# pdeljanov/Symphonia

Hardware: AMD Instinct MI355X
Metric: decoded audio frames/sec (batch IMDCT+OLA) (higher is better)
Workload: dtype f32

## Files before the change

symphonia_amd/build.py:

```python
import hashlib
import json
import os
import shutil
import subprocess
import sys
from pathlib import Path

HERE = Path(__file__).resolve().parent
CSRC = HERE / "csrc"
OUT = HERE / "libsymaccel.so"
TUNED_OUT = HERE / "build" / "tuned" / "libsymaccel.so"
SOURCES = ["tables.cpp", "ctx.cpp", "host_tools.cpp", "stage.cpp", "batcher.cpp", "multi.cpp", "imdct_generic.hip", "imdct_big.hip", "aac.hip", "aac_tools.hip", "mp3.hip", "mpa_polyphase.hip", "mp3_requant.hip",
           "mp3_stereo.hip", "vorbis.hip", "vorbis_wave.hip", "vorbis_wave2.hip", "vorbis_wg.hip", "flac.hip", "alac.hip", "state_copy.hip", "batch_copy.hip", "probe.hip"]
ARCH = "gfx950"
FLAGS = ["-O3", "-std=c++17", "-fPIC", "-I", str(CSRC), "-ffp-contract=off", "-fno-fast-math", "-fno-slp-vectorize", "-Wall", "-Wno-unused-function",
         "-Wno-unused-variable", "-Wno-unused-but-set-variable", "-Wno-missing-braces"]
_ILP = ["-mllvm", "-amdgpu-sched-strategy=iterative-ilp"]
SOURCE_FLAGS = {"aac_tools.hip": _ILP, "mp3.hip": _ILP, "alac.hip": _ILP, "flac.hip": _ILP}
TUNING_KNOBS = ("AAC_MIN_WAVES", "AAC_PREFETCH", "AAC_VARIANT", "NT", "MP3_WAVES", "MP3_VARIANT", "MP3_WG_WAVES", "MP3_FUSED_WAVES", "MP3_FUSED_WG_WAVES", "VORBIS_WAVES", "ALAC_SMALL_WAVES", "FLAC_PARTS", "MP3_SLOT_GROUP", "MP3_PACKED", "MP3_PAIR_GROUP", "AAC_ABLATE", "AAC_SINK", "AAC_CLOCK", "AAC_QUAD", "MULTI_WAVE", "VORBIS_WAVE2", "VORBIS_WG", "VORBIS_WG_SHARED", "ST_POLICY", "PACKED_C32", "WG4096_ABLATE", "FLAC_STORE_SWITCH", "ALAC_ONE_LAUNCH", "MP3_FRONT", "LDS_ABLATE", "F1_ABLATE", "F1_WAVES", "TNS_AHEAD", "TNS_ABLATE", "ALAC_UPDATE", "FLAC_OLDEST_FIRST", "FLAC_GROUP", "ALAC_UNROLL", "F1_LANE16", "FLAC_WAVES")
TUNE_PREFIX = "SYMACCEL_TUNE_"


def hipcc():
    exe = shutil.which("hipcc") or "/opt/rocm/bin/hipcc"
    if not Path(exe).exists():
        raise RuntimeError("hipcc not found: libsymaccel has no CPU build")
    return exe


def tuned_source_flags(env=None):
    env = os.environ if env is None else env
    names = [n for n in env.get(TUNE_PREFIX + "ILP", "").split(",") if n]
    for n in names:
        if n not in SOURCES:
            raise ValueError("%sILP names %r, not one of the sources" % (TUNE_PREFIX, n))
    out = {k: list(v) for k, v in SOURCE_FLAGS.items()}
    for n in names:
        out[n] = ["-mllvm", "-amdgpu-sched-strategy=" + env.get(TUNE_PREFIX + "SCHED", "iterative-ilp")]
    return out


def tuning_defines(env=None):
# ... 115 lines not shown
```

symphonia_amd/csrc/aac.hip:

```cpp
#include <type_traits>

#include "imdct_wave.h"

namespace symaccel {

namespace {

#ifndef SYM_AAC_VARIANT
#define SYM_AAC_VARIANT 0
#endif
#if SYM_AAC_VARIANT == 1
constexpr int kWaves = 6;
#define SYM_AAC_WAVES_PER_SIMD 3
#else
constexpr int kWaves = 4;
#endif
constexpr int kTabTw = 0;
constexpr int kTabKbd = 1024;
constexpr int kTabSine = 2048;
constexpr int kTabKbdShort = 3072;
constexpr int kTabSineShort = 3200;
constexpr int kTabFloats = 3328;

enum : int { ONLY_LONG = 0, LONG_START = 1, EIGHT_SHORT = 2, LONG_STOP = 3 };
constexpr int kP0 = 512 - 64;
constexpr int kP1 = 512 + 64;

__device__ __forceinline__ void pcm_short4(const float *H, int q0, const float *short_win, const float *prev_short_win,
                                           float (&acc)[4]) {
    const int w = q0 >> 7, i0 = q0 & 127;
    bool have = false;
    if (w >= 1) {
        float a[4];
        ys4(H, w - 1, 128 + i0, a);
        const float4 wr = *reinterpret_cast<const float4 *>(short_win + 124 - i0);
        a[0] *= wr.w; a[1] *= wr.z; a[2] *= wr.y; a[3] *= wr.x;
#pragma unroll
        for (int q = 0; q < 4; ++q) acc[q] = (w - 1 == 0) ? a[q] : (0.0f + a[q]);
        have = true;
    }
    if (w <= 7) {
        float bq[4];
        ys4(H, w, i0, bq);
        const float4 wf = *reinterpret_cast<const float4 *>((w == 0 ? prev_short_win : short_win) + i0);
        bq[0] *= wf.x; bq[1] *= wf.y; bq[2] *= wf.z; bq[3] *= wf.w;
#pragma unroll
        for (int q = 0; q < 4; ++q) acc[q] = have ? (acc[q] + bq[q]) : bq[q];
    }
}

__device__ __forceinline__ void stop_window4(const float *psw, int j0, float *w) {
    float4 v = make_float4(1.0f, 1.0f, 1.0f, 1.0f);
    if (j0 >= kP0 && j0 < kP1) v = *reinterpret_cast<const float4 *>(psw + j0 - kP0);
    w[0] = v.x; w[1] = v.y; w[2] = v.z; w[3] = v.w;
}
__device__ __forceinline__ void start_window4(const float *sw, int j0, float *w) {
    float4 v = make_float4(1.0f, 1.0f, 1.0f, 1.0f);
    if (j0 >= kP0 && j0 < kP1) {
        const float4 r = *reinterpret_cast<const float4 *>(sw + 124 - (j0 - kP0));
        v = make_float4(r.w, r.z, r.y, r.x);
    }
    w[0] = v.x; w[1] = v.y; w[2] = v.z; w[3] = v.w;
}

#if defined(SYM_AAC_WAVES_PER_SIMD) && !defined(SYM_AAC_MIN_WAVES)
#define SYM_AAC_MIN_WAVES SYM_AAC_WAVES_PER_SIMD
#endif
#ifndef SYM_AAC_MIN_WAVES
#define SYM_AAC_MIN_WAVES 2
#endif
#ifndef SYM_AAC_PREFETCH
#define SYM_AAC_PREFETCH 1
#endif
#ifndef SYM_AAC_QUAD
#define SYM_AAC_QUAD 1
#endif
__device__ __forceinline__ float2 ld_line(const float2 *p) { return ld_stream(p); }
__device__ __forceinline__ void st_slot(float *frame, int m2, const float (&v)[8]) {
    float4 *o4 = reinterpret_cast<float4 *>(frame);
    st_stream(o4 + m2, make_float4(v[0], v[1], v[2], v[3]));
    st_stream(o4 + 255 - m2, make_float4(v[4], v[5], v[6], v[7]));
}


#if !SYM_AAC_QUAD
#include "experiments/aac_wave_walk.h"
#endif



constexpr int kSlotOff = kShortRowsEnd;
static_assert(kSlotOff + 1024 <= kWaveLds, "delay slot must fit the per-wave LDS behind the short-window rows");

enum : int { kStepHalo = 0, kStepFull = 1, kStepRagged = 2 };
template <int V> using step_kind = std::integral_constant<int, V>;

__device__ __forceinline__ void settle_prefetch(const float2 (&line)[8]) {
#if defined(__HIP_DEVICE_COMPILE__)
    __builtin_amdgcn_sched_barrier(0);
    asm volatile("" : : "v"(line[0].x), "v"(line[0].y), "v"(line[1].x), "v"(line[1].y), "v"(line[2].x), "v"(line[2].y), "v"(line[3].x), "v"(line[3].y),
                        "v"(line[4].x), "v"(line[4].y), "v"(line[5].x), "v"(line[5].y), "v"(line[6].x), "v"(line[6].y), "v"(line[7].x), "v"(line[7].y));
#endif
}

struct AacJsArgs {
    const int2 *chain;
    const int32_t *pair_chains;
    const symaccel_aac_js_frame *desc;
    AacBandMaps maps;
    unsigned n_chains;
};

#if SYM_AAC_QUAD == 2
#include "experiments/aac_quad_probe.h"
#endif

template <bool JS>
__global__ __launch_bounds__(256, SYM_AAC_MIN_WAVES) void aac_synth_quad_kernel(
    DevTables tb, const float *__restrict__ coeffs, const uint8_t *__restrict__ side,
    const float *__restrict__ delay_in, float *__restrict__ delay_out, float *__restrict__ pcm,
    unsigned frames_per_chain, unsigned seg_steps, unsigned segs_per_chain, AacJsArgs js) {
    __shared__ __attribute__((aligned(16))) float tabs[kTabFloats];
    __shared__ __attribute__((aligned(16))) float wave_lds[4][kWaveLds];
    constexpr int CH = JS ? 2 : 1;
    __shared__ __attribute__((aligned(16))) float carry[CH][2][1024];
    if constexpr (!JS) {
        if (js.chain && js.chain[blockIdx.x / segs_per_chain].x >= 0) return;
    }
    for (int i = (int)threadIdx.x; i < 1024; i += 256) {
        tabs[kTabTw + i] = reinterpret_cast<const float *>(tb.aac_tw_long)[i];
        tabs[kTabKbd + i] = tb.aac_kbd_long[i];
        tabs[kTabSine + i] = tb.aac_sine_long[i];
        if (i < 128) {
            tabs[kTabKbdShort + i] = tb.aac_kbd_short[i];
// ... 260 lines not shown
            }
#pragma unroll
            for (int h = 0; h < 2; ++h) st_slot(frame_out, lane + 64 * h, dst[h]);
            if constexpr (KIND == kStepFull && !JS) settle_prefetch(line);
            if (t + 1 == (long)frames_per_chain) {
                float4 *d = reinterpret_cast<float4 *>(delay_out + (size_t)(ch ? chain1 : chain) * 1024);
#pragma unroll
                for (int q = 0; q < 4; ++q) d[lane + 64 * q] = reinterpret_cast<const float4 *>(my_slot)[lane + 64 * q];
            }
        }
        wg_sync_lds();
        }
        }
    };

    if (has_halo && wave == 3) step(step_kind<kStepHalo>{}, -1, t_begin - 1, true);
    if constexpr (!JS) settle_prefetch(line);
    const int n_full = (int)((t_end - t_begin) >> 2);
    long t = t_begin + wave;
#pragma unroll 1
    for (int i = 0; i < n_full; ++i, t += 4) step(step_kind<kStepFull>{}, i, t, true);
    if ((t_end - t_begin) & 3) step(step_kind<kStepRagged>{}, n_full, t, t < t_end);
}

__global__ void aac_js_index_kernel(const int32_t *__restrict__ pair_chains, unsigned n_pairs, unsigned n_chains, int2 *__restrict__ chain_index) {
    const unsigned i = blockIdx.x * blockDim.x + threadIdx.x;
    if (i < 2 * n_pairs && (unsigned)pair_chains[i] < n_chains && (unsigned)pair_chains[i ^ 1u] < n_chains)
        chain_index[pair_chains[i]] = make_int2(pair_chains[i ^ 1u], (int)i);
}

}

int launch_aac(symaccel_ctx *ctx, const float *d_coeffs, const uint8_t *d_side, const float *d_delay_in,
               float *d_delay_out, float *d_pcm, size_t n_chains, size_t frames_per_chain, const AacBandMaps *maps,
               const int32_t *d_pair_chains, const symaccel_aac_js_frame *d_js_desc, size_t n_pairs, void *d_js_scratch) {
    if (frames_per_chain > 0x7fffffffu) return SYMACCEL_ERR_INVALID_ARG;
#if SYM_AAC_QUAD
    {
        const size_t steps_per_chain = (frames_per_chain + 3) / 4;
        unsigned seg_steps;
        if (ctx->segment > 0) seg_steps = (unsigned)((ctx->segment + 3) / 4);
        else seg_steps = choose_segment(ctx, n_chains, steps_per_chain, SYM_AAC_MIN_WAVES, 1, 1, 1);
        if (seg_steps > steps_per_chain) seg_steps = (unsigned)steps_per_chain;
        const size_t segs = (steps_per_chain + seg_steps - 1) / seg_steps;
        const size_t grid = n_chains * segs;
        if (grid > 0x7fffffffu) return SYMACCEL_ERR_INVALID_ARG;
        AacJsArgs js{nullptr, nullptr, nullptr, AacBandMaps{}, (unsigned)n_chains};
        if (n_pairs == 0 || !maps) {
            hipLaunchKernelGGL(aac_synth_quad_kernel<false>, dim3((unsigned)grid), dim3(256), 0, ctx->stream, ctx->dev, d_coeffs, d_side,
                               d_delay_in, d_delay_out, d_pcm, (unsigned)frames_per_chain, seg_steps, (unsigned)segs, js);
        } else {
            if (n_pairs * frames_per_chain > 0x7fffffffu) return SYMACCEL_ERR_INVALID_ARG;
            const bool unpaired = 2 * n_pairs < n_chains;
            int2 *chain_index = unpaired ? reinterpret_cast<int2 *>(d_js_scratch) : nullptr;
            if (unpaired) {
                SYM_GPU(ctx, hipMemsetAsync(chain_index, 0xff, n_chains * sizeof(int2), ctx->stream));
                hipLaunchKernelGGL(aac_js_index_kernel, dim3((unsigned)((2 * n_pairs + 255) / 256)), dim3(256), 0, ctx->stream, d_pair_chains,
                                   (unsigned)n_pairs, (unsigned)n_chains, chain_index);
                SYM_GPU(ctx, hipGetLastError());
            }
            js = AacJsArgs{chain_index, d_pair_chains, d_js_desc, *maps, (unsigned)n_chains};
            unsigned pseg_steps;
            if (ctx->segment > 0) pseg_steps = (unsigned)((ctx->segment + 3) / 4);
            else pseg_steps = choose_segment(ctx, n_pairs, steps_per_chain, SYM_AAC_MIN_WAVES, 1, 1, 1);
            if (pseg_steps > steps_per_chain) pseg_steps = (unsigned)steps_per_chain;
            const size_t psegs = (steps_per_chain + pseg_steps - 1) / pseg_steps;
            if (n_pairs * psegs > 0x7fffffffu) return SYMACCEL_ERR_INVALID_ARG;
            hipLaunchKernelGGL(aac_synth_quad_kernel<true>, dim3((unsigned)(n_pairs * psegs)), dim3(256), 0, ctx->stream, ctx->dev, d_coeffs, d_side,
                               d_delay_in, d_delay_out, d_pcm, (unsigned)frames_per_chain, pseg_steps, (unsigned)psegs, js);
            SYM_GPU(ctx, hipGetLastError());
            if (unpaired)
                hipLaunchKernelGGL(aac_synth_quad_kernel<false>, dim3((unsigned)grid), dim3(256), 0, ctx->stream, ctx->dev, d_coeffs, d_side,
                                   d_delay_in, d_delay_out, d_pcm, (unsigned)frames_per_chain, seg_steps, (unsigned)segs, js);
        }
        SYM_GPU(ctx, hipGetLastError());
        return SYMACCEL_OK;
    }
#else
    return launch_aac_wave_walk(ctx, d_coeffs, d_side, d_delay_in, d_delay_out, d_pcm, n_chains, frames_per_chain);
#endif
}

}
```

symphonia_amd/csrc/aac_tools.hip:

```cpp
#include <hip/hip_runtime.h>

#include <cstdlib>

#include "symaccel_internal.h"

namespace symaccel {

namespace {

__global__ __launch_bounds__(256) void aac_joint_stereo_kernel(AacBandMaps maps, float *__restrict__ coeffs,
                                                               unsigned frames_per_chain, const int32_t *__restrict__ pair_chains,
                                                               const symaccel_aac_js_frame *__restrict__ desc,
                                                               const uint32_t *__restrict__ list, unsigned n_pair_frames) {
    const unsigned pf = list ? list[blockIdx.x] : blockIdx.x;
    if (pf >= n_pair_frames) return;
    const unsigned pair = pf / frames_per_chain, f = pf % frames_per_chain;
    const symaccel_aac_js_frame &d = desc[pf];
    const int t = (int)threadIdx.x;
    int sfb, slot;
    if (d.num_windows == 1) {
        sfb = maps.long4[t];
        slot = sfb;
    } else {
        sfb = maps.short4[t & 31];
        slot = (t >> 5) * 16 + sfb;
    }
    if (sfb >= (int)d.max_sfb || slot >= 128) return;
// ... 459 lines not shown
    }
}

template <bool DIRECT>
__global__ __launch_bounds__(128) void aac_tns_kernel(float *__restrict__ coeffs, unsigned n_frames, const symaccel_aac_tns_filter *__restrict__ filters,
                                                      unsigned n_filters, float *__restrict__ sink) {
    const unsigned wave = threadIdx.x >> 6, lane = threadIdx.x & 63u;
    const unsigned idx0 = blockIdx.x * 128u + lane, idx1 = idx0 + 64u;
    const int order0 = tns_filter_order(filters, idx0, n_filters, n_frames), order1 = tns_filter_order(filters, idx1, n_filters, n_frames);
    const int max_order = wave_max(order0 > order1 ? order0 : order1);
    if (max_order == 0) return;
    if (max_order > 12) {
        float lpc[kTnsMaxOrder];
        const TnsLane L = tns_lane<kTnsMaxOrder>(coeffs, filters, wave ? idx1 : idx0, wave ? order1 : order0, lpc);
        tns_walk<kTnsMaxOrder>(coeffs, L, lpc, wave_max(L.len), (int)lane);
        return;
    }
    if (wave != 0) return;
    if (max_order > 8) tns_pair_block<12, DIRECT>(coeffs, filters, sink, idx0, idx1, order0, order1, (int)lane);
    else if (max_order > 4) tns_pair_block<8, DIRECT>(coeffs, filters, sink, idx0, idx1, order0, order1, (int)lane);
    else tns_pair_block<4, DIRECT>(coeffs, filters, sink, idx0, idx1, order0, order1, (int)lane);
}

}

int launch_aac_joint_stereo(symaccel_ctx *ctx, const AacBandMaps &maps, float *d_coeffs, size_t frames_per_chain,
                            const int32_t *d_pair_chains, const symaccel_aac_js_frame *d_desc, size_t n_pairs, const uint32_t *d_list,
                            size_t n_list) {
    const size_t all = n_pairs * frames_per_chain;
    const size_t grid = d_list ? n_list : all;
    if (all > 0x7fffffffu || grid > 0x7fffffffu || frames_per_chain > 0xffffffffu) return SYMACCEL_ERR_INVALID_ARG;
    if (grid == 0) return SYMACCEL_OK;
    hipLaunchKernelGGL(aac_joint_stereo_kernel, dim3((unsigned)grid), dim3(256), 0, ctx->stream, maps, d_coeffs,
                       (unsigned)frames_per_chain, d_pair_chains, d_desc, d_list, (unsigned)all);
    SYM_GPU(ctx, hipGetLastError());
    return SYMACCEL_OK;
}

int launch_aac_js_consume(symaccel_ctx *ctx, symaccel_aac_js_frame *d_desc, const uint32_t *d_list, size_t n_list, size_t n_pair_frames) {
    if (n_list == 0) return SYMACCEL_OK;
    if (n_list > 0x7fffffffu || n_pair_frames > 0x7fffffffu) return SYMACCEL_ERR_INVALID_ARG;
    hipLaunchKernelGGL(aac_js_consume_kernel, dim3((unsigned)((n_list + 255) / 256)), dim3(256), 0, ctx->stream, d_desc, d_list,
                       (unsigned)n_list, (unsigned)n_pair_frames);
    SYM_GPU(ctx, hipGetLastError());
    return SYMACCEL_OK;
}
// ... 23 lines not shown
```

symphonia_amd/csrc/ctx.cpp:

```cpp
#include <cstring>
#include <new>

#include "symaccel_internal.h"

using namespace symaccel;

namespace symaccel {

int ctx_fail(symaccel_ctx *ctx, hipError_t err, const char *where) {
    if (ctx) {
        ctx->last_error = std::string(where) + ": " + hipGetErrorString(err);
    }
    return err == hipErrorOutOfMemory ? SYMACCEL_ERR_OOM : SYMACCEL_ERR_DEVICE;
}

int ctx_alloc(symaccel_ctx *ctx, void **out, size_t bytes, bool tracked) {
    *out = nullptr;
    if (bytes == 0) bytes = 16;
    SYM_GPU(ctx, hipMalloc(out, bytes));
    if (tracked) ctx->allocations.push_back(*out);
    return SYMACCEL_OK;
}

int ctx_sink(symaccel_ctx *ctx, void **out) {
// ... 217 lines not shown
}

const char *symaccel_last_error(const symaccel_ctx *ctx) { return ctx ? ctx->last_error.c_str() : ""; }

int symaccel_ctx_create(int device, symaccel_ctx **out) {
    if (!out) return SYMACCEL_ERR_INVALID_ARG;
    *out = nullptr;
    int count = 0;
    if (hipGetDeviceCount(&count) != hipSuccess || count <= 0) return SYMACCEL_ERR_DEVICE;
    if (device < 0 || device >= count) return SYMACCEL_ERR_INVALID_ARG;
    symaccel_ctx *ctx = new (std::nothrow) symaccel_ctx();
    if (!ctx) return SYMACCEL_ERR_OOM;
    ctx->device = device;
    int st = SYMACCEL_OK;
    int prev_device = -1;
    if (hipGetDevice(&prev_device) != hipSuccess) prev_device = -1;
    if (hipSetDevice(device) != hipSuccess || hipStreamCreate(&ctx->own_stream) != hipSuccess) {
        st = SYMACCEL_ERR_DEVICE;
    } else {
        ctx->stream = ctx->own_stream;
        int cus = 0;
        if (hipDeviceGetAttribute(&cus, hipDeviceAttributeMultiprocessorCount, device) == hipSuccess && cus > 0)
            ctx->n_cus = cus;
        st = upload_tables(ctx);
    }
    if (st != SYMACCEL_OK) {
        symaccel_ctx_destroy(ctx);
    } else {
        *out = ctx;
    }
    if (prev_device >= 0 && prev_device != device) (void)hipSetDevice(prev_device);
    return st;
}

void symaccel_ctx_destroy(symaccel_ctx *ctx) {
    if (!ctx) return;
    int prev_device = -1;
    if (hipGetDevice(&prev_device) != hipSuccess) prev_device = -1;
    (void)hipSetDevice(ctx->device);
    if (ctx->stream) (void)hipStreamSynchronize(ctx->stream);
    for (void *p : ctx->allocations) (void)hipFree(p);
    if (ctx->scratch) (void)hipFree(ctx->scratch);
    if (ctx->stage_in) (void)hipStreamSynchronize(ctx->stage_in);
    if (ctx->stage_out) (void)hipStreamSynchronize(ctx->stage_out);
    if (ctx->stage_arena) (void)hipFree(ctx->stage_arena);
    if (ctx->alac_flags) (void)hipFree(ctx->alac_flags);
// ... 1246 lines not shown
```

symphonia_amd/csrc/symaccel_internal.h:

```cpp
#pragma once

#include <cstddef>
#include <cstdint>
#include <map>
#include <string>
#include <utility>
#include <vector>

#include "../../include/symaccel.h"
#include <hip/hip_runtime.h>

namespace symaccel {

struct cpx {
    float re, im;
};

constexpr int kMp3Pow2abMinE = -1300, kMp3Pow2abLen = 1346;
constexpr int kMp3Unscaled = 39;

struct HostTables {
    std::vector<float> aac_kbd_long, aac_kbd_short, aac_sine_long, aac_sine_short;
    std::vector<cpx> aac_tw_long, aac_tw_short;
    std::vector<cpx> fft_merge;
// ... 60 lines not shown

constexpr int kMpa12Classes = 17;
enum Mpa12Layout {
    MPA12_FACTOR = 0,
    MPA12_SCF = 16,
    MPA12_CLASS = 80,
    MPA12_TOTAL = 131
};
constexpr int mpa12_n_frames(int layer) { return layer == SYMACCEL_MPA_LAYER1 ? 12 : layer == SYMACCEL_MPA_LAYER2 ? 36 : 0; }

struct ImdctPlan {
    int n;
    cpx *d_twiddle;
};

}

struct symaccel_ctx {
    int device = 0;
    hipStream_t stream = nullptr;
    hipStream_t own_stream = nullptr;
    int segment = 0;
    int n_cus = 256;
    std::string last_error;
    symaccel::DevTables dev{};
    std::vector<void *> allocations;
    std::map<std::pair<int, uint64_t>, symaccel::ImdctPlan> imdct_plans;
    std::map<int, float *> vorbis_windows;
    void *scratch = nullptr;
    size_t scratch_bytes = 0;
    hipStream_t stage_in = nullptr, stage_out = nullptr;
    hipEvent_t stage_events[6] = {nullptr, nullptr, nullptr, nullptr, nullptr, nullptr};
    void *stage_arena = nullptr;
    size_t stage_arena_bytes = 0;
    void *sink = nullptr;
    void *alac_flags = nullptr;
    size_t alac_flags_bytes = 0;
};

namespace symaccel {

int ctx_fail(symaccel_ctx *ctx, hipError_t err, const char *where);
int ctx_alloc(symaccel_ctx *ctx, void **out, size_t bytes, bool tracked = true);
int ctx_scratch(symaccel_ctx *ctx, size_t bytes, void **out);
constexpr size_t kSinkBytes = 2u << 20;
int ctx_sink(symaccel_ctx *ctx, void **out);
// ... 94 lines not shown
#define SYM_VORBIS_WG_SHARED 1
#endif
int launch_vorbis_wg(symaccel_ctx *ctx, int bs0_exp, int bs1_exp, const cpx *tw_short, const cpx *tw_long, const float *win_short,
                     const float *win_long, const float *d_spectra, const float *d_residue, size_t spec_stride, const uint8_t *d_block_flag,
                     const int32_t *d_prev_in, int32_t *d_prev_out, const float *d_overlap_in, float *d_overlap_out, float *d_pcm,
                     size_t pcm_stride, size_t n_chains, unsigned nb, unsigned seg, int floor_mode);
int launch_vorbis_wave2(symaccel_ctx *ctx, int bs0_exp, int bs1_exp, const cpx *tw_short, const cpx *tw_long, const float *win_short,
                        const float *win_long, const float *d_spectra, const float *d_residue, size_t spec_stride,
                        const uint8_t *d_block_flag, const int32_t *d_prev_in, int32_t *d_prev_out, const float *d_overlap_in,
                        float *d_overlap_out, float *d_pcm, size_t pcm_stride, size_t n_chains, unsigned nb, unsigned seg, int floor_mode);
int launch_vorbis_coupling(symaccel_ctx *ctx, float *d_mag, float *d_ang, size_t n);
int launch_vorbis_prepare(symaccel_ctx *ctx, float *d_residue, size_t spec_stride, unsigned channels_per_stream, size_t n_streams,
                          size_t blocks, const uint32_t *d_block_off, const uint8_t *d_steps, const uint32_t *d_step_first,
                          const uint8_t *d_kill);
int launch_vorbis_dot(symaccel_ctx *ctx, float *d_floor, const float *d_residue, size_t total);
int launch_vorbis_deinterleave(symaccel_ctx *ctx, const float *d_type2, float *d_planar, int n_ch, size_t n2,
                               size_t count);
int launch_vorbis_floor1(symaccel_ctx *ctx, const uint32_t *h_setup, int n_posts, int multiplier,
                         const uint32_t *d_y, uint32_t n, float *d_floor, size_t count, const float *d_residue = nullptr,
                         uint8_t *d_floor_y = nullptr, const uint32_t *d_line_offs = nullptr);
int launch_vorbis_floor1_pair(symaccel_ctx *ctx, const uint32_t *const h_setup[2], const int n_posts[2], const int multiplier[2],
                              const uint32_t *const d_y[2], const uint32_t n[2], const size_t count[2], const uint32_t *const d_line_offs[2],
                              uint8_t *d_floor_y);
int launch_aac_joint_stereo(symaccel_ctx *ctx, const AacBandMaps &maps, float *d_coeffs, size_t frames_per_chain,
                            const int32_t *d_pair_chains, const symaccel_aac_js_frame *d_desc, size_t n_pairs,
                            const uint32_t *d_list = nullptr, size_t n_list = 0);
int launch_aac_js_consume(symaccel_ctx *ctx, symaccel_aac_js_frame *d_desc, const uint32_t *d_list, size_t n_list, size_t n_pair_frames);
bool aac_band_maps(const uint16_t *swb_long, int n_swb_long, const uint16_t *swb_short, int n_swb_short, AacBandMaps *maps);
int launch_aac_tns(symaccel_ctx *ctx, float *d_coeffs, size_t n_frames, const symaccel_aac_tns_filter *d_filters,
                   size_t n_filters);
int launch_mp3_decode(symaccel_ctx *ctx, const int16_t *d_quant, const symaccel_mp3_requant *d_rq_desc, const int32_t *d_pair_chains,
                      const symaccel_mp3_stereo *d_st_desc, size_t n_pairs, const symaccel_mp3_side *d_side, int sr,
                      const float *d_overlap_in, const float *d_vvec_in, const int32_t *d_vfront_in, float *d_overlap_out,
                      float *d_vvec_out, int32_t *d_vfront_out, float *d_pcm, size_t n_chains, size_t granules_per_chain);
int launch_mp3_stereo(symaccel_ctx *ctx, float *d_xr, size_t granules_per_chain, const int32_t *d_pair_chains,
                      const symaccel_mp3_stereo *d_desc, int sr, size_t n_pairs, const int16_t *d_quant = nullptr,
                      const symaccel_mp3_requant *d_rq_desc = nullptr);
int launch_mp3_requantize(symaccel_ctx *ctx, const int16_t *d_quant, const symaccel_mp3_requant *d_desc, int sr,
                          float *d_xr, size_t n);
int launch_mpa_polyphase(symaccel_ctx *ctx, int n_frames, const float *d_in, const float *d_vvec_in,
                         const int32_t *d_vfront_in, float *d_vvec_out, int32_t *d_vfront_out, float *d_pcm, size_t n_chains,
                         size_t packets_per_chain);
int launch_mpa12_decode(symaccel_ctx *ctx, int layer, const uint16_t *d_codes, const uint8_t *d_rec, uint8_t *d_status,
                        const float *d_vvec_in, const int32_t *d_vfront_in, float *d_vvec_out, int32_t *d_vfront_out, float *d_pcm,
                        size_t n_chains, size_t packets_per_chain);
int launch_alac_predict(symaccel_ctx *ctx, int32_t *d_buf, const symaccel_alac_desc *d_desc, const int32_t *d_coeffs,
// ... 134 lines not shown
```

Measured before the change: 329.1 million.

## Add eight-wave paired-channel AAC walk kernel sharing joint-stereo data through LDS

Adds a new kernel in which one 512-thread workgroup decodes both channels of a stereo pair. Four waves work on each channel and exchange spectral lines through LDS, so M/S and intensity stereo can be applied inline. The kernel uses about 135 KB of LDS, so only one workgroup fits per CU, and it is selected by default when the device reports enough LDS per workgroup. The segment chooser is then asked for one wave per SIMD, which trades occupancy for less channel traffic and fewer separate stages.

Result: no change. 333.9 million (median of 2 runs) (+1.4%).

```diff
diff --git a/symphonia_amd/build.py b/symphonia_amd/build.py
--- a/symphonia_amd/build.py
+++ b/symphonia_amd/build.py
@@ -17,7 +17,7 @@
          "-Wno-unused-variable", "-Wno-unused-but-set-variable", "-Wno-missing-braces"]
 _ILP = ["-mllvm", "-amdgpu-sched-strategy=iterative-ilp"]
 SOURCE_FLAGS = {"aac_tools.hip": _ILP, "mp3.hip": _ILP, "alac.hip": _ILP, "flac.hip": _ILP}
-TUNING_KNOBS = ("AAC_MIN_WAVES", "AAC_PREFETCH", "AAC_VARIANT", "NT", "MP3_WAVES", "MP3_VARIANT", "MP3_WG_WAVES", "MP3_FUSED_WAVES", "MP3_FUSED_WG_WAVES", "VORBIS_WAVES", "ALAC_SMALL_WAVES", "FLAC_PARTS", "MP3_SLOT_GROUP", "MP3_PACKED", "MP3_PAIR_GROUP", "AAC_ABLATE", "AAC_SINK", "AAC_CLOCK", "AAC_QUAD", "MULTI_WAVE", "VORBIS_WAVE2", "VORBIS_WG", "VORBIS_WG_SHARED", "ST_POLICY", "PACKED_C32", "WG4096_ABLATE", "FLAC_STORE_SWITCH", "ALAC_ONE_LAUNCH", "MP3_FRONT", "LDS_ABLATE", "F1_ABLATE", "F1_WAVES", "TNS_AHEAD", "TNS_ABLATE", "ALAC_UPDATE", "FLAC_OLDEST_FIRST", "FLAC_GROUP", "ALAC_UNROLL", "F1_LANE16", "FLAC_WAVES")
+TUNING_KNOBS = ("AAC_MIN_WAVES", "AAC_PREFETCH", "AAC_VARIANT", "NT", "MP3_WAVES", "MP3_VARIANT", "MP3_WG_WAVES", "MP3_FUSED_WAVES", "MP3_FUSED_WG_WAVES", "VORBIS_WAVES", "ALAC_SMALL_WAVES", "FLAC_PARTS", "MP3_SLOT_GROUP", "MP3_PACKED", "MP3_PAIR_GROUP", "AAC_ABLATE", "AAC_SINK", "AAC_CLOCK", "AAC_QUAD", "MULTI_WAVE", "VORBIS_WAVE2", "VORBIS_WG", "VORBIS_WG_SHARED", "ST_POLICY", "PACKED_C32", "WG4096_ABLATE", "FLAC_STORE_SWITCH", "ALAC_ONE_LAUNCH", "MP3_FRONT", "LDS_ABLATE", "F1_ABLATE", "F1_WAVES", "TNS_AHEAD", "TNS_ABLATE", "ALAC_UPDATE", "FLAC_OLDEST_FIRST", "FLAC_GROUP", "ALAC_UNROLL", "F1_LANE16", "FLAC_WAVES", "AAC_PAIR8")
 TUNE_PREFIX = "SYMACCEL_TUNE_"
 
 
diff --git a/symphonia_amd/csrc/aac.hip b/symphonia_amd/csrc/aac.hip
--- a/symphonia_amd/csrc/aac.hip
+++ b/symphonia_amd/csrc/aac.hip
@@ -1,6 +1,7 @@
 #include <type_traits>
 
 #include "imdct_wave.h"
+#include "aac_walk.h"
 
 namespace symaccel {
 
@@ -15,54 +16,6 @@
 #else
 constexpr int kWaves = 4;
 #endif
-constexpr int kTabTw = 0;
-constexpr int kTabKbd = 1024;
-constexpr int kTabSine = 2048;
-constexpr int kTabKbdShort = 3072;
-constexpr int kTabSineShort = 3200;
-constexpr int kTabFloats = 3328;
-
-enum : int { ONLY_LONG = 0, LONG_START = 1, EIGHT_SHORT = 2, LONG_STOP = 3 };
-constexpr int kP0 = 512 - 64;
-constexpr int kP1 = 512 + 64;
-
-__device__ __forceinline__ void pcm_short4(const float *H, int q0, const float *short_win, const float *prev_short_win,
-                                           float (&acc)[4]) {
-    const int w = q0 >> 7, i0 = q0 & 127;
-    bool have = false;
-    if (w >= 1) {
-        float a[4];
-        ys4(H, w - 1, 128 + i0, a);
-        const float4 wr = *reinterpret_cast<const float4 *>(short_win + 124 - i0);
-        a[0] *= wr.w; a[1] *= wr.z; a[2] *= wr.y; a[3] *= wr.x;
-#pragma unroll
-        for (int q = 0; q < 4; ++q) acc[q] = (w - 1 == 0) ? a[q] : (0.0f + a[q]);
-        have = true;
-    }
-    if (w <= 7) {
-        float bq[4];
-        ys4(H, w, i0, bq);
-        const float4 wf = *reinterpret_cast<const float4 *>((w == 0 ? prev_short_win : short_win) + i0);
-        bq[0] *= wf.x; bq[1] *= wf.y; bq[2] *= wf.z; bq[3] *= wf.w;
-#pragma unroll
-        for (int q = 0; q < 4; ++q) acc[q] = have ? (acc[q] + bq[q]) : bq[q];
-    }
-}
-
-__device__ __forceinline__ void stop_window4(const float *psw, int j0, float *w) {
-    float4 v = make_float4(1.0f, 1.0f, 1.0f, 1.0f);
-    if (j0 >= kP0 && j0 < kP1) v = *reinterpret_cast<const float4 *>(psw + j0 - kP0);
-    w[0] = v.x; w[1] = v.y; w[2] = v.z; w[3] = v.w;
-}
-__device__ __forceinline__ void start_window4(const float *sw, int j0, float *w) {
-    float4 v = make_float4(1.0f, 1.0f, 1.0f, 1.0f);
-    if (j0 >= kP0 && j0 < kP1) {
-        const float4 r = *reinterpret_cast<const float4 *>(sw + 124 - (j0 - kP0));
-        v = make_float4(r.w, r.z, r.y, r.x);
-    }
-    w[0] = v.x; w[1] = v.y; w[2] = v.z; w[3] = v.w;
-}
-
 #if defined(SYM_AAC_WAVES_PER_SIMD) && !defined(SYM_AAC_MIN_WAVES)
 #define SYM_AAC_MIN_WAVES SYM_AAC_WAVES_PER_SIMD
 #endif
@@ -75,41 +28,13 @@
 #ifndef SYM_AAC_QUAD
 #define SYM_AAC_QUAD 1
 #endif
-__device__ __forceinline__ float2 ld_line(const float2 *p) { return ld_stream(p); }
-__device__ __forceinline__ void st_slot(float *frame, int m2, const float (&v)[8]) {
-    float4 *o4 = reinterpret_cast<float4 *>(frame);
-    st_stream(o4 + m2, make_float4(v[0], v[1], v[2], v[3]));
-    st_stream(o4 + 255 - m2, make_float4(v[4], v[5], v[6], v[7]));
-}
-
-
 #if !SYM_AAC_QUAD
 #include "experiments/aac_wave_walk.h"
 #endif
 
 
 
-constexpr int kSlotOff = kShortRowsEnd;
-static_assert(kSlotOff + 1024 <= kWaveLds, "delay slot must fit the per-wave LDS behind the short-window rows");
-
-enum : int { kStepHalo = 0, kStepFull = 1, kStepRagged = 2 };
-template <int V> using step_kind = std::integral_constant<int, V>;
-
-__device__ __forceinline__ void settle_prefetch(const float2 (&line)[8]) {
-#if defined(__HIP_DEVICE_COMPILE__)
-    __builtin_amdgcn_sched_barrier(0);
-    asm volatile("" : : "v"(line[0].x), "v"(line[0].y), "v"(line[1].x), "v"(line[1].y), "v"(line[2].x), "v"(line[2].y), "v"(line[3].x), "v"(line[3].y),
-                        "v"(line[4].x), "v"(line[4].y), "v"(line[5].x), "v"(line[5].y), "v"(line[6].x), "v"(line[6].y), "v"(line[7].x), "v"(line[7].y));
-#endif
-}
-
-struct AacJsArgs {
-    const int2 *chain;
-    const int32_t *pair_chains;
-    const symaccel_aac_js_frame *desc;
-    AacBandMaps maps;
-    unsigned n_chains;
-};
+
 
 #if SYM_AAC_QUAD == 2
 #include "experiments/aac_quad_probe.h"
@@ -416,6 +341,10 @@
     for (int i = 0; i < n_full; ++i, t += 4) step(step_kind<kStepFull>{}, i, t, true);
     if ((t_end - t_begin) & 3) step(step_kind<kStepRagged>{}, n_full, t, t < t_end);
 }
+
+#ifndef SYM_AAC_PAIR8
+#define SYM_AAC_PAIR8 1
+#endif
 
 __global__ void aac_js_index_kernel(const int32_t *__restrict__ pair_chains, unsigned n_pairs, unsigned n_chains, int2 *__restrict__ chain_index) {
     const unsigned i = blockIdx.x * blockDim.x + threadIdx.x;
@@ -454,14 +383,19 @@
                 SYM_GPU(ctx, hipGetLastError());
             }
             js = AacJsArgs{chain_index, d_pair_chains, d_js_desc, *maps, (unsigned)n_chains};
+            const bool pair8 = SYM_AAC_PAIR8 && ctx->lds_per_workgroup >= kAacPairLdsBytes;
             unsigned pseg_steps;
             if (ctx->segment > 0) pseg_steps = (unsigned)((ctx->segment + 3) / 4);
-            else pseg_steps = choose_segment(ctx, n_pairs, steps_per_chain, SYM_AAC_MIN_WAVES, 1, 1, 1);
+            else pseg_steps = choose_segment(ctx, n_pairs, steps_per_chain, pair8 ? 1 : SYM_AAC_MIN_WAVES, 1, 1, 1);
             if (pseg_steps > steps_per_chain) pseg_steps = (unsigned)steps_per_chain;
             const size_t psegs = (steps_per_chain + pseg_steps - 1) / pseg_steps;
             if (n_pairs * psegs > 0x7fffffffu) return SYMACCEL_ERR_INVALID_ARG;
-            hipLaunchKernelGGL(aac_synth_quad_kernel<true>, dim3((unsigned)(n_pairs * psegs)), dim3(256), 0, ctx->stream, ctx->dev, d_coeffs, d_side,
-                               d_delay_in, d_delay_out, d_pcm, (unsigned)frames_per_chain, pseg_steps, (unsigned)psegs, js);
+            if (pair8)
+                launch_aac_pair_walk(ctx, d_coeffs, d_side, d_delay_in, d_delay_out, d_pcm, (unsigned)frames_per_chain, pseg_steps, (unsigned)psegs,
+                                     (unsigned)n_pairs, d_pair_chains, d_js_desc, *maps, (unsigned)n_chains);
+            else
+                hipLaunchKernelGGL(aac_synth_quad_kernel<true>, dim3((unsigned)(n_pairs * psegs)), dim3(256), 0, ctx->stream, ctx->dev, d_coeffs, d_side,
+                                   d_delay_in, d_delay_out, d_pcm, (unsigned)frames_per_chain, pseg_steps, (unsigned)psegs, js);
             SYM_GPU(ctx, hipGetLastError());
             if (unpaired)
                 hipLaunchKernelGGL(aac_synth_quad_kernel<false>, dim3((unsigned)grid), dim3(256), 0, ctx->stream, ctx->dev, d_coeffs, d_side,
diff --git a/symphonia_amd/csrc/aac_pair.hip b/symphonia_amd/csrc/aac_pair.hip
--- /dev/null
+++ b/symphonia_amd/csrc/aac_pair.hip
@@ -0,0 +1,306 @@
+constexpr int kPairWaves = 8;
+constexpr int kPairTwShort = 128;
+constexpr int kPairLdsBytes = 4 * (kTabFloats + kPairTwShort + kPairWaves * kWaveLds + 2 * 2 * 1024 + kPairWaves * 1024);
+static_assert(kPairLdsBytes == kAacPairLdsBytes && kPairLdsBytes <= 160 * 1024, "the pair walk's LDS: one workgroup per CU");
+
+__device__ __forceinline__ void settle_pair_prefetch(const float2 (&line)[8], const uint32_t (&dq)[3], unsigned sb) {
+#if defined(__HIP_DEVICE_COMPILE__)
+    __builtin_amdgcn_sched_barrier(0);
+    asm volatile("" : : "v"(line[0].x), "v"(line[0].y), "v"(line[1].x), "v"(line[1].y), "v"(line[2].x), "v"(line[2].y), "v"(line[3].x), "v"(line[3].y),
+                        "v"(line[4].x), "v"(line[4].y), "v"(line[5].x), "v"(line[5].y), "v"(line[6].x), "v"(line[6].y), "v"(line[7].x), "v"(line[7].y),
+                        "v"(dq[0]), "v"(dq[1]), "v"(dq[2]), "v"(sb));
+#endif
+}
+
+__global__ __launch_bounds__(512, 2) void aac_pair_walk_kernel(
+    DevTables tb, const float *__restrict__ coeffs, const uint8_t *__restrict__ side,
+    const float *__restrict__ delay_in, float *__restrict__ delay_out, float *__restrict__ pcm,
+    unsigned frames_per_chain, unsigned seg_steps, unsigned segs_per_chain, AacJsArgs js) {
+    __shared__ __attribute__((aligned(16))) float tabs[kTabFloats];
+    __shared__ __attribute__((aligned(16))) float tw_short[kPairTwShort];
+    __shared__ __attribute__((aligned(16))) float wave_lds[kPairWaves][kWaveLds];
+    __shared__ __attribute__((aligned(16))) float carry[2][2][1024];
+    __shared__ __attribute__((aligned(16))) float2 xchg[kPairWaves][512];
+    const int lane = (int)threadIdx.x & 63, wave = __builtin_amdgcn_readfirstlane((int)threadIdx.x >> 6);
+    const int ch = wave >> 2, wj = wave & 3;
+    float *ldsf = wave_lds[wave];
+    c32 *lds = reinterpret_cast<c32 *>(ldsf);
+    const c32 *tw = reinterpret_cast<const c32 *>(tabs + kTabTw);
+    const unsigned unit = blockIdx.x / segs_per_chain, seg = blockIdx.x % segs_per_chain;
+    const unsigned chain_l = (unsigned)js.pair_chains[2 * unit], chain_r = (unsigned)js.pair_chains[2 * unit + 1];
+    if (chain_l >= js.n_chains || chain_r >= js.n_chains || chain_l == chain_r) return;
+    const unsigned chain = ch ? chain_r : chain_l;
+    const long t_begin = (long)seg * seg_steps * 4;
+    const long t_end = t_begin + (long)seg_steps * 4 < (long)frames_per_chain ? t_begin + (long)seg_steps * 4 : (long)frames_per_chain;
+    if (t_end <= t_begin) return;
+    const size_t chain_base = (size_t)chain * frames_per_chain;
+    const symaccel_aac_js_frame *desc = js.desc + (size_t)unit * frames_per_chain;
+    const bool has_halo = t_begin > 0;
+
+    float2 line[8];
+    uint32_t dq[3] = {0u, 0u, 0u};
+    unsigned sb_next = 0;
+    auto request = [&](long tf) __attribute__((always_inline)) {
+        const uint32_t *d = reinterpret_cast<const uint32_t *>(desc + (size_t)tf);
+        const float2 *src = reinterpret_cast<const float2 *>(coeffs + (chain_base + (size_t)tf) * 1024);
+        sb_next = side[chain_base + (size_t)tf];
+        dq[0] = d[lane];
+        dq[1] = d[lane + 64];
+        dq[2] = lane < 33 ? d[lane + 128] : 0u;
+#pragma unroll
+        for (int s = 0; s < 8; ++s) line[s] = ld_line(src + lane + 64 * s);
+    };
+    const long t_first = (wj == 3 && has_halo) ? t_begin - 1 : t_begin + wj;
+    if (t_first < t_end) {
+        request(t_first);
+    } else {
+#pragma unroll
+        for (int s = 0; s < 8; ++s) line[s] = make_float2(0.0f, 0.0f);
+    }
+    for (int i = (int)threadIdx.x; i < 1024; i += 64 * kPairWaves) {
+        tabs[kTabTw + i] = reinterpret_cast<const float *>(tb.aac_tw_long)[i];
+        tabs[kTabKbd + i] = tb.aac_kbd_long[i];
+        tabs[kTabSine + i] = tb.aac_sine_long[i];
+        if (i < 128) {
+            tabs[kTabKbdShort + i] = tb.aac_kbd_short[i];
+            tabs[kTabSineShort + i] = tb.aac_sine_short[i];
+            tw_short[i] = reinterpret_cast<const float *>(tb.aac_tw_short)[i];
+        }
+    }
+    LaneTables lt;
+    load_lane_tables(tb, lane, lt);
+    if (!has_halo && wj == 3) {
+        const float4 *src = reinterpret_cast<const float4 *>(delay_in + (size_t)chain * 1024);
+#pragma unroll
+        for (int q = 0; q < 4; ++q) reinterpret_cast<float4 *>(carry[ch][1])[lane + 64 * q] = src[lane + 64 * q];
+    }
+    uint32_t sfb_long[2] = {0u, 0u};
+#pragma unroll
+    for (int s = 0; s < 8; ++s) {
+        const uint32_t b = js.maps.long4[(lane >> 1) + 32 * s];
+        sfb_long[s >> 2] |= (b < 128u ? b : 128u) << (8 * (s & 3));
+    }
+    const unsigned sfb_short = js.maps.short4[(lane >> 1) & 31] < 128u ? js.maps.short4[(lane >> 1) & 31] : 128u;
+
+    auto publish = [&]() __attribute__((always_inline)) {
+#pragma unroll
+        for (int s = 0; s < 8; ++s) xchg[wave][lane + 64 * s] = line[s];
+    };
+    auto pick = [](unsigned mask, float a, float b) __attribute__((always_inline)) {
+        return __uint_as_float((__float_as_uint(a) & mask) | (__float_as_uint(b) & ~mask));
+    };
+    auto decode_lines = [&](auto one_c, auto right_c, unsigned max_sfb, const float2 (&other)[8], const uint8_t *mode, const float *scale) __attribute__((always_inline)) {
+        constexpr bool ONE = decltype(one_c)::value;
+        constexpr bool RIGHT = decltype(right_c)::value;
+        const unsigned lim = max_sfb < 128u ? max_sfb : 128u;
+#pragma unroll
+        for (int s = 0; s < 8; ++s) {
+            const float2 mine = line[s];
+            const unsigned sfb = ONE ? (sfb_long[s >> 2] >> (8 * (s & 3))) & 255u : sfb_short;
+            const unsigned slot = ONE ? sfb : 16u * (unsigned)s + sfb;
+            const unsigned coded = (unsigned)(sfb < lim) & (unsigned)(slot < 128u);
+            const unsigned m = mode[slot];
+            const unsigned ms = 0u - (coded & (unsigned)(m == SYMACCEL_AAC_JS_MS));
+            if constexpr (!RIGHT) {
+                line[s] = make_float2(pick(ms, mine.x + other[s].x, mine.x), pick(ms, mine.y + other[s].y, mine.y));
+            } else {
+                const unsigned is = 0u - (coded & (unsigned)(m == SYMACCEL_AAC_JS_INTENSITY));
+                const float sc = scale[slot];
+                line[s] = make_float2(pick(ms, other[s].x - mine.x, pick(is, sc * other[s].x, mine.x)),
+                                      pick(ms, other[s].y - mine.y, pick(is, sc * other[s].y, mine.y)));
+            }
+        }
+    };
+    auto decode = [&]() __attribute__((always_inline)) {
+        uint32_t *dl = reinterpret_cast<uint32_t *>(ldsf);
+        dl[lane] = dq[0];
+        if (ch) {
+            dl[lane + 64] = dq[1];
+            if (lane < 33) dl[lane + 128] = dq[2];
+        }
+        wave_sync();
+        float2 other[8];
+#pragma unroll
+        for (int s = 0; s < 8; ++s) other[s] = xchg[wave ^ 4][lane + 64 * s];
+        const unsigned hdr = (unsigned)__builtin_amdgcn_readfirstlane((int)dl[0]);
+        const unsigned max_sfb = (hdr >> 8) & 255u;
+        const uint8_t *mode = reinterpret_cast<const uint8_t *>(dl + 1);
+        const float *scale = reinterpret_cast<const float *>(dl + 33);
+        const bool one = (hdr & 255u) == 1u;
+        if (ch == 0) {
+            if (one) decode_lines(std::true_type{}, std::false_type{}, max_sfb, other, mode, scale);
+            else decode_lines(std::false_type{}, std::false_type{}, max_sfb, other, mode, scale);
+        } else {
+            if (one) decode_lines(std::true_type{}, std::true_type{}, max_sfb, other, mode, scale);
+            else decode_lines(std::false_type{}, std::true_type{}, max_sfb, other, mode, scale);
+        }
+        wave_sync();
+    };
+
+    publish();
+    __syncthreads();
+    decode();
+
+    auto step = [&](auto kind_c, int i, long t, bool active) __attribute__((always_inline)) {
+        constexpr int KIND = decltype(kind_c)::value;
+        const unsigned sb = (unsigned)__builtin_amdgcn_readfirstlane((int)sb_next);
+        const long tn = KIND == kStepHalo ? t_begin + 3 : (t + 4 < t_end ? t + 4 : t);
+        const bool fetch = KIND == kStepFull || (KIND == kStepHalo && active && tn < t_end);
+        const int seq = (int)(sb & 3u);
+        const int shape = (int)((sb >> 2) & 1u), prev_shape = (int)((sb >> 3) & 1u);
+        float *my_slot = wj == 3 ? carry[ch][i & 1] : ldsf + kSlotOff;
+        float *prev_slot = wj == 0 ? carry[ch][(i + 1) & 1] : wave_lds[wave > 0 ? wave - 1 : 0] + kSlotOff;
+        float xw[2][8];
+        auto long_tail = [&](auto seq_c) __attribute__((always_inline)) {
+            constexpr int SEQ = decltype(seq_c)::value;
+            const float *wprev = tabs + (prev_shape ? kTabKbd : kTabSine);
+            const float *wcur = tabs + (shape ? kTabKbd : kTabSine);
+#pragma unroll
+            for (int h = 0; h < 2; ++h) {
+                const int m2 = lane + 64 * h;
+                float x[8], x2[8];
+                post_slot(lds, tw, m2, x, x2);
+                float wo[8];
+                if constexpr (SEQ == LONG_STOP) {
+                    const float *psw = tabs + (prev_shape ? kTabKbdShort : kTabSineShort);
+                    stop_window4(psw, 4 * m2, wo);
+                    stop_window4(psw, 1020 - 4 * m2, wo + 4);
+                } else {
+                    load_slot(wprev, m2, wo);
+                }
+#pragma unroll
+                for (int q = 0; q < 8; ++q) xw[h][q] = x[q] * wo[q];
+                float wd[8], nd[8];
+                if constexpr (SEQ == LONG_START) {
+                    const float *sw = tabs + (shape ? kTabKbdShort : kTabSineShort);
+                    start_window4(sw, 4 * m2, wd);
+                    start_window4(sw, 1020 - 4 * m2, wd + 4);
+                } else {
+                    float wr[8];
+                    if (SEQ == ONLY_LONG && shape == prev_shape) {
+#pragma unroll
+                        for (int q = 0; q < 8; ++q) wr[q] = wo[q];
+                    } else {
+                        load_slot(wcur, m2, wr);
+                    }
+#pragma unroll
+                    for (int q = 0; q < 8; ++q) wd[q] = wr[7 - q];
+                }
+#pragma unroll
+                for (int q = 0; q < 8; ++q) {
+                    const int j = q < 4 ? 4 * m2 + q : 1020 - 4 * m2 + (q - 4);
+                    const float v = x2[q] * wd[q];
+                    nd[q] = (SEQ == LONG_START && j >= kP1) ? 0.0f : v;
+                }
+                store_slot(my_slot, m2, nd);
+            }
+        };
+
+        if (active) {
+            c32 z[8];
+            if (seq != EIGHT_SHORT) {
+                const int mirror = (63 - lane) * 4;
+#pragma unroll
+                for (int s = 0; s < 8; ++s) {
+                    const float mirrored = __int_as_float(__builtin_amdgcn_ds_bpermute(mirror, __float_as_int(line[7 - s].y)));
+                    z[s] = pre_twiddle(line[s].x, mirrored, tw[lane + 64 * s]);
+                }
+            } else {
+#pragma unroll
+                for (int s = 0; s < 8; ++s) {
+                    ldsf[short_row(s) + 2 * lane] = line[s].x;
+                    ldsf[short_row(s) + 2 * lane + 1] = line[s].y;
+                }
+                wave_sync();
+            }
+            if (fetch) request(tn);
+            if (seq != EIGHT_SHORT) {
+                fft512_wave(z, lane, lds, lt);
+                if (seq == ONLY_LONG) long_tail(step_kind<ONLY_LONG>{});
+                else if (seq == LONG_START) long_tail(step_kind<LONG_START>{});
+                else long_tail(step_kind<LONG_STOP>{});
+            } else {
+                imdct_short_wave(lane, ldsf, reinterpret_cast<const cpx *>(tw_short), lt);
+                const float *sw = tabs + (shape ? kTabKbdShort : kTabSineShort);
+                const float *psw = tabs + (prev_shape ? kTabKbdShort : kTabSineShort);
+#pragma unroll 1
+                for (int e = 0; e < 4; ++e) {
+                    const int j0 = 4 * lane + 256 * e;
+                    float nd[4] = {0.0f, 0.0f, 0.0f, 0.0f};
+                    if (j0 < kP1) pcm_short4(ldsf, j0 + kP1, sw, psw, nd);
+                    *reinterpret_cast<float4 *>(my_slot + j0) = make_float4(nd[0], nd[1], nd[2], nd[3]);
+                }
+            }
+        }
+        wg_sync_lds();
+
+        if constexpr (KIND == kStepHalo) {
+            if (fetch) {
+                settle_pair_prefetch(line, dq, sb_next);
+                publish();
+            }
+        } else if (active) {
+            float *frame_out = pcm + (chain_base + (size_t)t) * 1024;
+            float dst[2][8];
+            if (seq != EIGHT_SHORT) {
+#pragma unroll
+                for (int h = 0; h < 2; ++h) {
+                    const int m2 = lane + 64 * h;
+                    float dl[8];
+                    load_slot(prev_slot, m2, dl);
+#pragma unroll
+                    for (int q = 0; q < 8; ++q) dst[h][q] = dl[q] + xw[h][q];
+                    if (seq == LONG_STOP) {
+#pragma unroll
+                        for (int q = 0; q < 8; ++q) {
+                            const int j = q < 4 ? 4 * m2 + q : 1020 - 4 * m2 + (q - 4);
+                            dst[h][q] = j < kP0 ? dl[q] : dst[h][q];
+                        }
+                    }
+                }
+            } else {
+                const float *sw = tabs + (shape ? kTabKbdShort : kTabSineShort);
+                const float *psw = tabs + (prev_shape ? kTabKbdShort : kTabSineShort);
+#pragma unroll 1
+                for (int e = 0; e < 4; ++e) {
+                    const int j0 = 4 * lane + 256 * e;
+                    const float4 d = *reinterpret_cast<const float4 *>(prev_slot + j0);
+                    float o[4] = {d.x, d.y, d.z, d.w};
+                    if (j0 >= kP0) {
+                        float ps[4];
+                        pcm_short4(ldsf, j0 - kP0, sw, psw, ps);
+#pragma unroll
+                        for (int q = 0; q < 4; ++q) o[q] = o[q] + ps[q];
+                    }
+                    *reinterpret_cast<float4 *>(prev_slot + j0) = make_float4(o[0], o[1], o[2], o[3]);
+                }
+                wave_sync();
+#pragma unroll
+                for (int h = 0; h < 2; ++h) load_slot(prev_slot, lane + 64 * h, dst[h]);
+            }
+#pragma unroll
+            for (int h = 0; h < 2; ++h) st_slot(frame_out, lane + 64 * h, dst[h]);
+            if constexpr (KIND == kStepFull) {
+                settle_pair_prefetch(line, dq, sb_next);
+                publish();
+            }
+            if (t + 1 == (long)frames_per_chain) {
+                float4 *d = reinterpret_cast<float4 *>(delay_out + (size_t)chain * 1024);
+#pragma unroll
+                for (int q = 0; q < 4; ++q) d[lane + 64 * q] = reinterpret_cast<const float4 *>(my_slot)[lane + 64 * q];
+            }
+        }
+        wg_sync_lds();
+        if (fetch) decode();
+    };
+
+    if (has_halo) {
+        step(step_kind<kStepHalo>{}, -1, t_begin - 1, wj == 3);
+        settle_pair_prefetch(line, dq, sb_next);
+    }
+    const int n_full = (int)((t_end - t_begin) >> 2);
+    long t = t_begin + wj;
+#pragma unroll 1
+    for (int i = 0; i < n_full; ++i, t += 4) step(step_kind<kStepFull>{}, i, t, true);
+    if ((t_end - t_begin) & 3) step(step_kind<kStepRagged>{}, n_full, t, t < t_end);
+}
diff --git a/symphonia_amd/csrc/aac_tools.hip b/symphonia_amd/csrc/aac_tools.hip
--- a/symphonia_amd/csrc/aac_tools.hip
+++ b/symphonia_amd/csrc/aac_tools.hip
@@ -3,6 +3,7 @@
 #include <cstdlib>
 
 #include "symaccel_internal.h"
+#include "aac_walk.h"
 
 namespace symaccel {
 
@@ -508,6 +509,16 @@
     else tns_pair_block<4, DIRECT>(coeffs, filters, sink, idx0, idx1, order0, order1, (int)lane);
 }
 
+#include "aac_pair.hip"
+
+}
+
+void launch_aac_pair_walk(symaccel_ctx *ctx, const float *d_coeffs, const uint8_t *d_side, const float *d_delay_in, float *d_delay_out, float *d_pcm,
+                          unsigned frames_per_chain, unsigned seg_steps, unsigned segs_per_chain, unsigned n_pairs, const int32_t *d_pair_chains,
+                          const symaccel_aac_js_frame *d_js_desc, const AacBandMaps &maps, unsigned n_chains) {
+    const AacJsArgs js{nullptr, d_pair_chains, d_js_desc, maps, n_chains};
+    hipLaunchKernelGGL(aac_pair_walk_kernel, dim3(n_pairs * segs_per_chain), dim3(64 * kPairWaves), 0, ctx->stream, ctx->dev, d_coeffs, d_side,
+                       d_delay_in, d_delay_out, d_pcm, frames_per_chain, seg_steps, segs_per_chain, js);
 }
 
 int launch_aac_joint_stereo(symaccel_ctx *ctx, const AacBandMaps &maps, float *d_coeffs, size_t frames_per_chain,
diff --git a/symphonia_amd/csrc/aac_walk.h b/symphonia_amd/csrc/aac_walk.h
--- /dev/null
+++ b/symphonia_amd/csrc/aac_walk.h
@@ -0,0 +1,89 @@
+#pragma once
+
+#include <type_traits>
+
+#include "imdct_wave.h"
+
+namespace symaccel {
+
+namespace {
+
+constexpr int kTabTw = 0;
+constexpr int kTabKbd = 1024;
+constexpr int kTabSine = 2048;
+constexpr int kTabKbdShort = 3072;
+constexpr int kTabSineShort = 3200;
+constexpr int kTabFloats = 3328;
+
+enum : int { ONLY_LONG = 0, LONG_START = 1, EIGHT_SHORT = 2, LONG_STOP = 3 };
+constexpr int kP0 = 512 - 64;
+constexpr int kP1 = 512 + 64;
+
+__device__ __forceinline__ void pcm_short4(const float *H, int q0, const float *short_win, const float *prev_short_win,
+                                           float (&acc)[4]) {
+    const int w = q0 >> 7, i0 = q0 & 127;
+    bool have = false;
+    if (w >= 1) {
+        float a[4];
+        ys4(H, w - 1, 128 + i0, a);
+        const float4 wr = *reinterpret_cast<const float4 *>(short_win + 124 - i0);
+        a[0] *= wr.w; a[1] *= wr.z; a[2] *= wr.y; a[3] *= wr.x;
+#pragma unroll
+        for (int q = 0; q < 4; ++q) acc[q] = (w - 1 == 0) ? a[q] : (0.0f + a[q]);
+        have = true;
+    }
+    if (w <= 7) {
+        float bq[4];
+        ys4(H, w, i0, bq);
+        const float4 wf = *reinterpret_cast<const float4 *>((w == 0 ? prev_short_win : short_win) + i0);
+        bq[0] *= wf.x; bq[1] *= wf.y; bq[2] *= wf.z; bq[3] *= wf.w;
+#pragma unroll
+        for (int q = 0; q < 4; ++q) acc[q] = have ? (acc[q] + bq[q]) : bq[q];
+    }
+}
+
+__device__ __forceinline__ void stop_window4(const float *psw, int j0, float *w) {
+    float4 v = make_float4(1.0f, 1.0f, 1.0f, 1.0f);
+    if (j0 >= kP0 && j0 < kP1) v = *reinterpret_cast<const float4 *>(psw + j0 - kP0);
+    w[0] = v.x; w[1] = v.y; w[2] = v.z; w[3] = v.w;
+}
+__device__ __forceinline__ void start_window4(const float *sw, int j0, float *w) {
+    float4 v = make_float4(1.0f, 1.0f, 1.0f, 1.0f);
+    if (j0 >= kP0 && j0 < kP1) {
+        const float4 r = *reinterpret_cast<const float4 *>(sw + 124 - (j0 - kP0));
+        v = make_float4(r.w, r.z, r.y, r.x);
+    }
+    w[0] = v.x; w[1] = v.y; w[2] = v.z; w[3] = v.w;
+}
+
+__device__ __forceinline__ float2 ld_line(const float2 *p) { return ld_stream(p); }
+__device__ __forceinline__ void st_slot(float *frame, int m2, const float (&v)[8]) {
+    float4 *o4 = reinterpret_cast<float4 *>(frame);
+    st_stream(o4 + m2, make_float4(v[0], v[1], v[2], v[3]));
+    st_stream(o4 + 255 - m2, make_float4(v[4], v[5], v[6], v[7]));
+}
+
+constexpr int kSlotOff = kShortRowsEnd;
+static_assert(kSlotOff + 1024 <= kWaveLds, "delay slot must fit the per-wave LDS behind the short-window rows");
+
+enum : int { kStepHalo = 0, kStepFull = 1, kStepRagged = 2 };
+template <int V> using step_kind = std::integral_constant<int, V>;
+
+__device__ __forceinline__ void settle_prefetch(const float2 (&line)[8]) {
+#if defined(__HIP_DEVICE_COMPILE__)
+    __builtin_amdgcn_sched_barrier(0);
+    asm volatile("" : : "v"(line[0].x), "v"(line[0].y), "v"(line[1].x), "v"(line[1].y), "v"(line[2].x), "v"(line[2].y), "v"(line[3].x), "v"(line[3].y),
+                        "v"(line[4].x), "v"(line[4].y), "v"(line[5].x), "v"(line[5].y), "v"(line[6].x), "v"(line[6].y), "v"(line[7].x), "v"(line[7].y));
+#endif
+}
+
+struct AacJsArgs {
+    const int2 *chain;
+    const int32_t *pair_chains;
+    const symaccel_aac_js_frame *desc;
+    AacBandMaps maps;
+    unsigned n_chains;
+};
+}
+
+}
diff --git a/symphonia_amd/csrc/ctx.cpp b/symphonia_amd/csrc/ctx.cpp
--- a/symphonia_amd/csrc/ctx.cpp
+++ b/symphonia_amd/csrc/ctx.cpp
@@ -263,6 +263,11 @@
         int cus = 0;
         if (hipDeviceGetAttribute(&cus, hipDeviceAttributeMultiprocessorCount, device) == hipSuccess && cus > 0)
             ctx->n_cus = cus;
+#if !defined(SYMACCEL_EMULATED_HIP)
+        int lds = 0;
+        if (hipDeviceGetAttribute(&lds, hipDeviceAttributeMaxSharedMemoryPerBlock, device) == hipSuccess && lds > 0)
+            ctx->lds_per_workgroup = lds;
+#endif
         st = upload_tables(ctx);
     }
     if (st != SYMACCEL_OK) {
diff --git a/symphonia_amd/csrc/symaccel_internal.h b/symphonia_amd/csrc/symaccel_internal.h
--- a/symphonia_amd/csrc/symaccel_internal.h
+++ b/symphonia_amd/csrc/symaccel_internal.h
@@ -106,6 +106,7 @@
     hipStream_t own_stream = nullptr;
     int segment = 0;
     int n_cus = 256;
+    int lds_per_workgroup = 160 * 1024;
     std::string last_error;
     symaccel::DevTables dev{};
     std::vector<void *> allocations;
@@ -246,6 +247,10 @@
 int launch_vorbis_floor1_pair(symaccel_ctx *ctx, const uint32_t *const h_setup[2], const int n_posts[2], const int multiplier[2],
                               const uint32_t *const d_y[2], const uint32_t n[2], const size_t count[2], const uint32_t *const d_line_offs[2],
                               uint8_t *d_floor_y);
+constexpr int kAacPairLdsBytes = 135424;
+void launch_aac_pair_walk(symaccel_ctx *ctx, const float *d_coeffs, const uint8_t *d_side, const float *d_delay_in, float *d_delay_out, float *d_pcm,
+                          unsigned frames_per_chain, unsigned seg_steps, unsigned segs_per_chain, unsigned n_pairs, const int32_t *d_pair_chains,
+                          const symaccel_aac_js_frame *d_js_desc, const AacBandMaps &maps, unsigned n_chains);
 int launch_aac_joint_stereo(symaccel_ctx *ctx, const AacBandMaps &maps, float *d_coeffs, size_t frames_per_chain,
                             const int32_t *d_pair_chains, const symaccel_aac_js_frame *d_desc, size_t n_pairs,
                             const uint32_t *d_list = nullptr, size_t n_list = 0);
```
